# galatolofederico/clip-glass

Hardware: AMD Instinct MI355X
Metric: candidate latents scored/sec (GAN→CLIP fitness), StyleGAN2_ffhq_d pop=64 (higher is better)
Workload: dtype f16; 1 GPU; StyleGAN2_ffhq_d: StyleGAN2 config-f 1024px G+D + CLIP ViT-B/32, pop=64 per GPU, batch_size=4, n_obj=2; pop_per_gpu=64, global_pop=64, batch_size=4, parallelism=population-shard x1, device=AMD Radeon Graphics (gfx950:sramecc+:xnack-), 256 CUs, hbm_gib=288

## Files before the change

### clip_glass_amd/csrc/conv_glds.hip

```cpp
#include "common.h"
#include "kernels.h"
#include <stdlib.h>
#include <type_traits>

namespace {
constexpr int NT = 128, NTHR = 512;
template <int TW>
struct Geo {
    static constexpr int RW = TW == 32 ? 2 : 1;
    static constexpr int TH = 8 * RW * (32 / TW);
    static constexpr int PH = TH + 2, PW = TW + 2;
    static constexpr int NVA = PH * PW * 4;
    static constexpr int NA = (NVA + NTHR - 1) / NTHR;
    static constexpr int A_BYTES = NA * NTHR * 16;
    static constexpr int OFF_B = 2 * A_BYTES;
    static constexpr int OFF_C = OFF_B + 3 * (3 * NT * 64);
    static constexpr int OFF_S = OFF_C + 3 * NT * 4;
    static constexpr int OFF_T = OFF_S + 2048;
    static constexpr int OFF_N = OFF_T + 6 * NT * 2 + 512;
    static constexpr int LDS_BYTES = OFF_N + 8 * 64 * 4;
    static_assert(LDS_BYTES <= 163840, "one workgroup per CU");
};
constexpr int NB = 3 * NT * 4 / NTHR;
constexpr int B_BYTES = 3 * NT * 64;
// ... 201 lines not shown
        for (int g = 0; g < 4; ++g) {
            const int nl = j * 32 + 8 * g + 4 * kh;
            const f4 d = *(const f4*)(Cc + nl), bb = *(const f4*)(Cc + NT + nl);
#pragma unroll
            for (int i = 0; i < RW; ++i) {
                const f4 a = {acc[i][j][g * 4], acc[i][j][g * 4 + 1], acc[i][j][g * 4 + 2], acc[i][j][g * 4 + 3]};
                f4 v = act_apply(a * d + bb + nzr[i], ak);
                if (p.res) v += f4{(float)rq[g][i][0], (float)rq[g][i][1], (float)rq[g][i][2], (float)rq[g][i][3]} * p.out_scale;
                h4 out;
#pragma unroll
                for (int q = 0; q < 4; ++q) out[q] = (half_t)v[q];
                *(h4*)(Os + (i * 32 + lr) * OROW + nl * 2) = out;
                if (TRGB) va[i][g] = out;
            }
        }
        if (TRGB) {
#pragma unroll
            for (int gp = 0; gp < 2; ++gp) {
                const h8 wt = *(const h8*)(Trow + ((j * 2 + gp) * 2) * 16);
#pragma unroll
                for (int i = 0; i < RW; ++i) {
                    const h8 wi = (trow_ok && ((tn >> 2) & 1) == i) ? wt : hzero;
                    rgb = mfma32(wi, __builtin_shufflevector(va[i][2 * gp], va[i][2 * gp + 1], 0, 1, 2, 3, 4, 5, 6, 7), rgb);
                }
            }
        }
    }
    if (TRGB) {
        const long long hw = (long long)p.Ho * p.Wo;
        float* yo = p.trgb_yout + (long long)b * 3 * hw + (long long)(oyb + kh) * p.Wo + ox;
#pragma unroll
        for (int c = 0; c < 3; ++c) {
            float r = p.trgb_b[c] + (rgb[c] + rgb[4 + c] * (1.f / 2048.f));
            if (p.trgb_yprev) r += trgb_skip(ytap[c], oyb + kh, ox);
            yo[c * hw] = r;
        }
    }
    __builtin_amdgcn_wave_barrier();
#pragma unroll
    for (int i = 0; i < RW; ++i) {
#pragma unroll
        for (int k = 0; k < NT / 16; ++k) {
            const int v = lane + 64 * k;
            const int pix = v >> 4, chv = v & 15;
            const int prow = TW == 32 ? 0 : pix >> 4, pcol = TW == 32 ? pix : pix & 15;
            half_t* dst = p.y + (((long long)b * p.Ho + ty0 + (wave * RW + i) * RPL + prow) * p.Wo + tx0 + pcol) * p.Cout + n0;
            *(h8*)(dst + chv * 8) = *(const h8*)(Os + (i * 32 + pix) * OROW + chv * 16);
        }
    }
}

template <bool TRGB, bool XS = false, bool ST = true>
__global__ __launch_bounds__(512, 1) void conv_gldsp_kernel(ConvParams p, int NTn, int tiles_x, int tiles_y, int PT) {
    constexpr int TW = 32;
    using G = Geo<TW>;
    constexpr int RW = G::RW, TH = G::TH, PW = G::PW, NVA = G::NVA, NA = G::NA, A_BYTES = G::A_BYTES, OFF_B = G::OFF_B,
                  OFF_C = G::OFF_C, OFF_S = G::OFF_S;
    static_assert(RW == 2 && 8 * RW * 32 * 80 <= A_BYTES, "the sliced output image fits one patch buffer");
    static_assert(NA == 5 && NB == 3, "ring pieces per phase: one weight piece per phase of a stage, one patch piece in phases 0..4 of a chunk");
    extern __shared__ __attribute__((aligned(16))) char smem[];
    const int wave = __builtin_amdgcn_readfirstlane(threadIdx.x >> 6);
    const int grp = wave >> 2;
    const int tpi = tiles_x * tiles_y;
    const int n_work = ((PT + 7) & ~7) * NTn;
    struct Item { int b, ty0, tx0, n0, valid; };
    auto decode = [&](int id) {
        Item w;
        const int lo = id & 7, rest = id >> 3;
        const int nt = rest % NTn, pt = (rest / NTn) * 8 + lo;
        w.valid = id < n_work && pt < PT;
        const int ptc = w.valid ? pt : 0;
        w.b = ptc / tpi;
        const int trem = ptc - w.b * tpi;
        w.ty0 = (trem / tiles_x) * TH;
        w.tx0 = (trem % tiles_x) * TW;
        w.n0 = nt * NT;
        return w;
    };
    int id = blockIdx.x;
    Item cur = decode(id);
    while (id < n_work && !cur.valid) { id += gridDim.x; cur = decode(id); }
    if (id >= n_work) return;

    const half_t* xb = p.x;
    const half_t* wb = p.w;
    int a_src[NA];
    int b_src[NB];
    auto aim_a = [&](const Item& w) {
        const int t = opaque(threadIdx.x);
        xb = p.x + (long long)w.b * p.x_bstride;
#pragma unroll
        for (int k = 0; k < NA; ++k) {
            const int v = k * NTHR + t, pix = v >> 2;
            const int pr = pix / PW, pc = pix - pr * PW;
            const int iy = w.ty0 - 1 + pr, ix = w.tx0 - 1 + pc;
            const int lc = (v & 3) ^ ((pix >> 2) & 3);
            const bool ok = v < NVA && iy >= 0 && iy < p.H && ix >= 0 && ix < p.W;
            a_src[k] = ok ? (iy * p.W + ix) * p.Cin + lc * 8 : -1;
        }
    };
    auto aim_b = [&](const Item& w) {
        const int t = opaque(threadIdx.x);
        wb = p.w + (long long)w.b * p.w_bstride;
#pragma unroll
        for (int k = 0; k < NB; ++k) {
            const int v = k * NTHR + t, row = v >> 2;
            const int tx = row >> 7, n = row & 127;
            const int lc = (v & 3) ^ ((row >> 2) & 3);
            b_src[k] = (tx * p.Neff + w.n0 + n) * p.Cin + lc * 8;
        }
    };
    auto issue_a1 = [&](int k, int c, int buf) {
        char* dst = smem + buf * A_BYTES + wave * 1024 + k * (NTHR * 16);
        dma16(a_src[k] >= 0 ? xb + a_src[k] + c * 32 : g_zero_page + (threadIdx.x & 3) * 8, dst);
    };
    auto issue_b1 = [&](int k, int c, int ty, int slot) {
        char* dst = smem + OFF_B + slot * B_BYTES + wave * 1024 + k * (NTHR * 16);
        dma16(wb + (long long)ty * 3 * p.Neff * p.Cin + c * 32 + b_src[k], dst);
    };
    const int n_chunks = p.Cin >> 5;
    const half_t* Ss = (const half_t*)(smem + OFF_S);
    auto park_style = [&](int b) {
        const int t = threadIdx.x;
        if (t < (p.Cin >> 3)) *(h8*)(smem + OFF_S + t * 16) = *(const h8*)(p.sn16 + (long long)b * p.sn_stride + t * 8);
    };

    aim_a(cur);
    aim_b(cur);
    if (p.sn16) park_style(cur.b);
    {
        const int t = threadIdx.x;
        float* Cc = (float*)(smem + OFF_C);
        if (t < NT) {
            if (!p.dscale) Cc[t] = 1.f;
            if (!p.bias) Cc[NT + t] = 0.f;
            if (!p.shift) Cc[2 * NT + t] = 0.f;
        }
        if (!p.noise) *(float*)(smem + G::OFF_N + t * 4) = 0.f;
    }
    __syncthreads();
#pragma unroll
    for (int k = 0; k < NA; ++k) issue_a1(k, 0, 0);
#pragma unroll
    for (int k = 0; k < NB; ++k) issue_b1(k, 0, 0, 0);
#pragma unroll
    for (int k = 0; k < NB; ++k) issue_b1(k, 0, 1, 1);
    WAIT_VM(3);
    __builtin_amdgcn_s_barrier();
    for (;;) {
        int nid = id + gridDim.x;
        Item nxt = decode(nid);
        while (nid < n_work && !nxt.valid) { nid += gridDim.x; nxt = decode(nid); }
        const bool has_next = nid < n_work;
        if (!has_next) nxt = cur;
        const int b = cur.b, ty0 = cur.ty0, tx0 = cur.tx0, n0 = cur.n0;

        f16x acc[RW][4];
#pragma unroll
        for (int i = 0; i < RW; ++i)
#pragma unroll
            for (int j = 0; j < 4; ++j)
#pragma unroll
                for (int q = 0; q < 16; ++q) acc[i][j][q] = 0.f;

        auto prefetch_epilogue = [&]() {
            const int t = opaque(threadIdx.x), lr = t & 31, kh = (t >> 5) & 1;
            if (wave < 2) {
                char* cc = smem + OFF_C + wave * 256;
                if (p.dscale) dma4(p.dscale + (long long)b * p.ds_stride + n0 + t, cc);
                if (p.bias) dma4(p.bias + n0 + t, cc + NT * 4);
                if (p.shift) dma4(p.shift + (long long)b * p.ds_stride + n0 + t, cc + 2 * NT * 4);
            }
            if (p.noise) dma4(p.noise + ((long long)(b / p.batch_size) * p.Ho + ty0 + wave * RW + kh) * p.Wo + tx0 + lr, smem + G::OFF_N + wave * 256);
            if (TRGB && wave < 2) {
                const int row6 = min(t / (NT / 8), 5), piece = t % (NT / 8);
                const int n = row6 < 3 ? row6 : 8 + (row6 - 3);
                dma16(t < 6 * (NT / 8) ? p.trgb_tab + ((long long)b * 32 + n) * p.Neff + n0 + piece * 8 : g_zero_page, smem + G::OFF_T + wave * 1024);
            }
        };
        if (grp) __builtin_amdgcn_s_barrier();
        auto chunk_body = [&](const int c, auto lastc_tag) {
            constexpr bool lastc = decltype(lastc_tag)::value;
            const char* As = smem + (c & 1) * A_BYTES;
#pragma unroll
            for (int ty = 0; ty < 3; ++ty) {
#pragma unroll
                for (int tx = 0; tx < 3; ++tx) {
                    const int q = ty * 3 + tx;
                    auto ring_pieces = [&]() {
                        if (q == 6 && lastc) prefetch_epilogue();
                        {
                            const int t2 = (ty + 2) % 3;
                            int c2 = ty == 0 ? c : c + 1;
                            if (ty != 0 && lastc) {
                                if (q == 3) aim_b(nxt);
                                c2 = 0;
                            }
                            issue_b1(tx, c2, t2, t2);
                        }
                        if (q < 5) {
                            if (q == 0 && lastc) aim_a(nxt);
                            issue_a1(q, lastc ? 0 : c + 1, lastc ? 0 : (c + 1) & 1);
                        }
                    };
                    if (XS && q == 0 && c % NTn == (n0 >> 7)) {
                        const int tq = opaque(threadIdx.x), part = tq & 3, pix = tq >> 2, ly = pix >> 4, lx = pix & 15;
                        h8 s03, s12;
                        h8 k125, k375;
#pragma unroll
                        for (int e = 0; e < 8; ++e) { k125[e] = (half_t)0.125f; k375[e] = (half_t)0.375f; }
#pragma unroll
                        for (int jy = 0; jy < 4; ++jy) {
                            h8 a[4];
#pragma unroll
                            for (int jx = 0; jx < 4; ++jx) {
                                const int P = (2 * ly + jy) * PW + 2 * lx + jx;
                                a[jx] = *(const h8*)(As + P * 64 + ((part ^ ((P >> 2) & 3)) << 4));
                            }
                            const h8 hr = __builtin_elementwise_fma(a[0] + a[3], k125, (a[1] + a[2]) * k375);
                            if (jy == 0) s03 = hr;
                            else if (jy == 1) s12 = hr;
                            else if (jy == 2) s12 = s12 + hr;
                            else s03 = s03 + hr;
                        }
                        const h8 o = __builtin_elementwise_fma(s12, k375, s03 * k125);
                        *(h8*)(p.xs_out + (((long long)b * (p.H >> 1) + (ty0 >> 1) + ly) * (p.W >> 1) + (tx0 >> 1) + lx) * p.Cin + c * 32 + part * 8) = o;
                    }
                    h8 wf[2][4], xf[2][RW];
                    {
                        const int tm = opaque(threadIdx.x), lr = tm & 31, kh = (tm >> 5) & 1;
                        const char* Bs = smem + OFF_B + ty * B_BYTES;
#pragma unroll
                        for (int kk = 0; kk < 2; ++kk) {
                            const int lc = kk * 2 + kh;
#pragma unroll
                            for (int j = 0; j < 4; ++j) {
                                const int row = tx * NT + j * 32 + lr;
                                wf[kk][j] = *(const h8*)(Bs + row * 64 + ((lc ^ ((row >> 2) & 3)) << 4));
                            }
#pragma unroll
                            for (int i = 0; i < RW; ++i) {
                                const int pix = (wave * RW + i + ty) * PW + lr + tx;
                                xf[kk][i] = *(const h8*)(As + pix * 64 + ((lc ^ ((pix >> 2) & 3)) << 4));
                            }
                            if (ST) {
                                const h8 sv = *(const h8*)(Ss + c * 32 + lc * 8);
#pragma unroll
                                for (int j = 0; j < 4; ++j) wf[kk][j] = wf[kk][j] * sv;
                            }
                        }
                    }
                    if (tx == 2) { if (ty == 2) WAIT_VM(2); else if (ty == 1) WAIT_VM(5); else WAIT_VM(4); }
                    asm volatile("s_waitcnt lgkmcnt(0)" ::: "memory");
                    __builtin_amdgcn_sched_barrier(0);
                    __builtin_amdgcn_s_barrier();
                    __builtin_amdgcn_s_setprio(1);
#pragma unroll
                    for (int kk = 0; kk < 2; ++kk)
#pragma unroll
                        for (int j = 0; j < 4; ++j) {
#pragma unroll
                            for (int i = 0; i < RW; ++i) acc[i][j] = mfma32(wf[kk][j], xf[kk][i], acc[i][j]);
                            if (kk == 0 && j == 1) { __builtin_amdgcn_sched_barrier(0); ring_pieces(); __builtin_amdgcn_sched_barrier(0); }
                        }
                    __builtin_amdgcn_s_setprio(0);
                    __builtin_amdgcn_sched_barrier(0);
                    __builtin_amdgcn_s_barrier();
                }
            }
        };
        for (int c = 0; c + 1 < n_chunks; ++c) chunk_body(c, std::false_type{});
        chunk_body(n_chunks - 1, std::true_type{});

        if (!grp) __builtin_amdgcn_s_barrier();
        const int t = opaque(threadIdx.x), lane = t & 63, lr = lane & 31, kh = lane >> 5;
        const float* Cc = (const float*)(smem + OFF_C);
        constexpr int OP = 80;
        char* Os = smem + A_BYTES + wave * (RW * 32 * OP);
        const int oyb = ty0 + wave * RW, ox = tx0 + lr;
        const int rcs = p.res_cs ? p.res_cs : p.Cout;
        const ActK ak = act_consts(p.act, p.out_scale);
        float ytap[3][4];
        h8 nsty;
        if (TRGB && p.trgb_yprev) {
            const int my = (oyb + kh) >> 1, mx = ox >> 1, h2 = p.Ho >> 1, w2 = p.Wo >> 1;
            const float* yp = p.trgb_yprev + (long long)b * 3 * h2 * w2;
#pragma unroll
            for (int cc = 0; cc < 3; ++cc)
#pragma unroll
                for (int q = 0; q < 4; ++q)
                    ytap[cc][q] = yp[(cc * h2 + max(my - 1 + (q >> 1), 0)) * w2 + max(mx - 1 + (q & 1), 0)];
        }
        if (ST && t < (p.Cin >> 3)) nsty = *(const h8*)(p.sn16 + (long long)nxt.b * p.sn_stride + t * 8);
        float nzr[RW];
#pragma unroll
        for (int i = 0; i < RW; ++i) nzr[i] = p.noise_strength * *(const float*)(smem + G::OFF_N + (wave * 64 + i * 32 + lr) * 4);
        f16x rgb;
#pragma unroll
        for (int q = 0; q < 16; ++q) rgb[q] = 0.f;
        const int tn = lr & 15;
        const char* Trow = smem + G::OFF_T + (((tn >> 3) & 1) * 3 + min(tn & 3, 2)) * (NT * 2) + kh * 16;
        const bool trow_ok = (tn & 3) < 3;
        const h8 hzero = {0, 0, 0, 0, 0, 0, 0, 0};
#pragma unroll
        for (int j = 0; j < 4; ++j) {
            h4 va[RW][4];
            h4 rq[4][RW];
            if (p.res) {
#pragma unroll
                for (int i = 0; i < RW; ++i) {
                    const int oy = oyb + i;
                    const half_t* rp = p.res + (p.res_up ? (((long long)b * (p.Ho >> 1) + (oy >> 1)) * (p.Wo >> 1) + (ox >> 1)) * rcs
                                                         : (((long long)b * p.Ho + oy) * p.Wo + ox) * rcs) + n0 + j * 32 + 4 * kh;
#pragma unroll
                    for (int g = 0; g < 4; ++g) rq[g][i] = *(const h4*)(rp + 8 * g);
                }
            }
            constexpr int GB = TRGB ? 2 : 4;
#pragma unroll
            for (int g0 = 0; g0 < 4; g0 += GB) {
            f4 dq[GB], bq[GB];
#pragma unroll
            for (int g = 0; g < GB; ++g) {
                const int nl = j * 32 + 8 * (g0 + g) + 4 * kh;
                dq[g] = *(const f4*)(Cc + nl);
                bq[g] = *(const f4*)(Cc + NT + nl) + *(const f4*)(Cc + 2 * NT + nl);
            }
            __builtin_amdgcn_sched_barrier(0);
#pragma unroll
            for (int g = g0; g < g0 + GB; ++g) {
                const f4 d = dq[g - g0], bb = bq[g - g0];
#pragma unroll
                for (int i = 0; i < RW; ++i) {
                    const f4 a = {acc[i][j][g * 4], acc[i][j][g * 4 + 1], acc[i][j][g * 4 + 2], acc[i][j][g * 4 + 3]};
                    f4 v = act_apply(a * d + bb + nzr[i], ak);
                    if (p.res) v += f4{(float)rq[g][i][0], (float)rq[g][i][1], (float)rq[g][i][2], (float)rq[g][i][3]} * p.out_scale;
                    h4 out;
#pragma unroll
                    for (int q = 0; q < 4; ++q) out[q] = (half_t)v[q];
                    *(h4*)(Os + (i * 32 + lr) * OP + (8 * g + 4 * kh) * 2) = out;
                    if (TRGB) va[i][g] = out;
                }
            }
            }
            if (TRGB) {
#pragma unroll
                for (int gp = 0; gp < 2; ++gp) {
                    const h8 wt = *(const h8*)(Trow + ((j * 2 + gp) * 2) * 16);
#pragma unroll
                    for (int i = 0; i < RW; ++i) {
                        const h8 wi = (trow_ok && ((tn >> 2) & 1) == i) ? wt : hzero;
                        rgb = mfma32(wi, __builtin_shufflevector(va[i][2 * gp], va[i][2 * gp + 1], 0, 1, 2, 3, 4, 5, 6, 7), rgb);
                    }
                }
            }
            __builtin_amdgcn_wave_barrier();
#pragma unroll
            for (int k = 0; k < 4; ++k) {
                const int v = lane + 64 * k, i = v >> 7, pix = (v >> 2) & 31, piece = v & 3;
                half_t* dst = p.y + (((long long)b * p.Ho + oyb + i) * p.Wo + tx0 + pix) * p.Cout + n0 + j * 32 + piece * 8;
                *(h8*)dst = *(const h8*)(Os + (i * 32 + pix) * OP + piece * 16);
            }
            __builtin_amdgcn_wave_barrier();
        }
        if (TRGB) {
            const long long hw = (long long)p.Ho * p.Wo;
            if (p.trgb_part) {
                float* yo = p.trgb_part + ((long long)(n0 >> 7) * p.B + b) * 3 * hw + (long long)(oyb + kh) * p.Wo + ox;
#pragma unroll
                for (int cc = 0; cc < 3; ++cc) yo[cc * hw] = rgb[cc] + rgb[4 + cc] * (1.f / 2048.f);
            } else {
                float* yo = p.trgb_yout + (long long)b * 3 * hw + (long long)(oyb + kh) * p.Wo + ox;
#pragma unroll
                for (int cc = 0; cc < 3; ++cc) {
                    float r = p.trgb_b[cc] + (rgb[cc] + rgb[4 + cc] * (1.f / 2048.f));
                    if (p.trgb_yprev) r += trgb_skip(ytap[cc], oyb + kh, ox);
                    yo[cc * hw] = r;
                }
            }
        }
        if (ST && t < (p.Cin >> 3)) *(h8*)(smem + OFF_S + t * 16) = nsty;
        asm volatile("s_waitcnt lgkmcnt(0)" ::: "memory");
        __builtin_amdgcn_s_barrier();
        if (!has_next) break;
        id = nid;
        cur = nxt;
    }
    WAIT_VM(0);
}


static constexpr uint32_t GLDS_FEATURES = CF_STYLE | CF_DEMOD | CF_SHIFT | CF_NOISE | CF_RES | CF_RES_CS | CF_RES_UP | CF_SAMPLE_W | CF_TORGB |
                                          CF_TORGB_PART | CF_XS_OUT;

static int glds_cus() { return glass_cu_count() - glass_cu_count() % 8; }
template <int TW, bool TRGB>
static void launch_glds(const ConvParams& p, hipStream_t st) {
    using G = Geo<TW>;
    static DevOnce once;
    once.run([&] { (void)hipFuncSetAttribute((const void*)conv_glds_kernel<TW, TRGB>, hipFuncAttributeMaxDynamicSharedMemorySize, G::LDS_BYTES); });
    const int tiles_x = p.Wc / TW, tiles_y = p.Hc / G::TH, PT = p.B * tiles_x * tiles_y, NTn = p.Neff / NT;
    hipLaunchKernelGGL((conv_glds_kernel<TW, TRGB>), dim3((PT + 7) / 8 * 8 * NTn), dim3(NTHR), G::LDS_BYTES, st, p, NTn, tiles_x, tiles_y, PT);
}
template <bool TRGB, bool XS, bool ST>
static void launch_gldsp(const ConvParams& p, hipStream_t st) {
    using G = Geo<32>;
    static DevOnce once;
    once.run([&] { (void)hipFuncSetAttribute((const void*)conv_gldsp_kernel<TRGB, XS, ST>, hipFuncAttributeMaxDynamicSharedMemorySize, G::LDS_BYTES); });
    const int tiles_x = p.Wc / 32, tiles_y = p.Hc / G::TH, PT = p.B * tiles_x * tiles_y, NTn = p.Neff / NT;
    hipLaunchKernelGGL((conv_gldsp_kernel<TRGB, XS, ST>), dim3(glds_cus()), dim3(NTHR), G::LDS_BYTES, st, p, NTn, tiles_x, tiles_y, PT);
}

template <int TW, bool TRGB = false>
static ConvKernel glds_inst(const ConvParams& p, const char* name) {
    const long long work_nominal = (long long)GLASS_NOMINAL_POP * (p.Wc / TW) * (p.Hc / Geo<TW>::TH) * (p.Neff / NT);
    if (TW == 32 && (p.Cin & 63) == 0 && work_nominal >= 2 * glds_cus()) {
        const bool sty = p.sn16 != nullptr;
        if (p.xs_out && !TRGB) return sty ? ConvKernel{"conv_gldsp_kernel<false,true,true>", launch_gldsp<false, true, true>}
                                          : ConvKernel{"conv_gldsp_kernel<false,true,false>", launch_gldsp<false, true, false>};
        if (TRGB) return sty ? ConvKernel{"conv_gldsp_kernel<true,false,true>", launch_gldsp<true, false, true>}
                             : ConvKernel{"conv_gldsp_kernel<true,false,false>", launch_gldsp<true, false, false>};
        return sty ? ConvKernel{"conv_gldsp_kernel<false,false,true>", launch_gldsp<false, false, true>}
                   : ConvKernel{"conv_gldsp_kernel<false,false,false>", launch_gldsp<false, false, false>};
    }
    if (p.xs_out || p.trgb_part) return conv_refused();
    return {name, launch_glds<TW, TRGB>};
}

ConvKernel choose_conv_glds(const ConvParams& p) {
    const uint32_t f = conv_features(p);
    if (f & ~GLDS_FEATURES) return conv_refused(f & ~GLDS_FEATURES);
    if (!glass_lds_fits(Geo<32>::LDS_BYTES) || !glass_lds_fits(Geo<16>::LDS_BYTES)) return conv_refused();
    if (((f & CF_XS_OUT) && ((f & (CF_STYLE | CF_TORGB | CF_TORGB_PART)) || p.Wc % 32 != 0)) || !p.y || p.KS != 3 || p.stride != 1 || p.pad != 1)
        return conv_refused();
    if (((f & CF_STYLE) && !p.sn16) || p.Cin > 1024) return conv_refused();
    if (p.Cin % 32 != 0 || p.Cin < 128 || p.Neff % NT != 0 || (p.Cout & 7) || p.Hc % 16 != 0) return conv_refused();
    if ((long long)p.H * p.W * p.Cin >= (1LL << 31)) return conv_refused();
    if (f & CF_TORGB_PART) {
        if (!p.trgb_tab || (f & CF_TORGB) || p.trgb_yprev || p.Neff != p.Cout || p.Wc % 32 != 0) return conv_refused();
        return glds_inst<32, true>(p, nullptr);
    }
    if (f & CF_TORGB) {
        if (!p.trgb_tab || !p.trgb_b || p.Neff != NT || p.Cout != NT || p.Wc % 32 != 0) return conv_refused();
        return glds_inst<32, true>(p, "conv_glds_kernel<32,true>");
    }
    if (p.Wc % 32 == 0) return glds_inst<32>(p, "conv_glds_kernel<32>");
    if (p.Wc % 16 == 0) return glds_inst<16>(p, "conv_glds_kernel<16>");
    return conv_refused();
}
```

### clip_glass_amd/csrc/conv_stream.hip

```cpp
#include "common.h"
#include "kernels.h"
#include <stdio.h>
#include <stdlib.h>

namespace {
constexpr int TH = 8, PH = TH + 2;
constexpr int W_BYTES = 9 * 32 * 64;
constexpr int PP = 36;
constexpr int A_BYTES = PH * PP * 64;
constexpr int O_BYTES = 4 * 32 * 64;
constexpr int C_BYTES = 32 * 4 + 32 * 4 + 32 * 2 + 4 * 32 * 2;
constexpr int LDS_BYTES = W_BYTES + A_BYTES + O_BYTES + C_BYTES;
__device__ __forceinline__ int swz(int row, int chunk) { return (row << 6) + ((chunk ^ ((row >> 2) & 3)) << 4); }
__device__ __forceinline__ int opaque(int v) { asm volatile("" : "+v"(v)); return v; }
__device__ __forceinline__ int swa(int pr, int pc, int chunk) { return ((pr * PP + pc) << 6) + ((chunk ^ ((pc >> 2) & 3)) << 4); }
}

template <bool FRGB, bool TRGB, bool TR = false>
__global__ __launch_bounds__(256, 3) void conv_stream_kernel(ConvParams p, int tiles_x, int tiles_y, int PT, int per_block) {
    static_assert(!TR, "placeholder of a removed experiment");
    extern __shared__ __attribute__((aligned(16))) char smem[];
    char* Ws = smem;
    char* As = smem + W_BYTES;
    const int t = threadIdx.x;
    float* Cd = (float*)(smem + W_BYTES + A_BYTES + O_BYTES);
    float* Cb = Cd + 32;
    half_t* Cs = (half_t*)(Cb + 32);
    half_t* Cf = Cs + 32;
    char* Tw = smem + W_BYTES + A_BYTES;
    float* Ys = (float*)(Tw + 2048);
    float* Tb = Ys + 256;
    if (FRGB) {
        if (t < 32) {
            Cf[t] = (half_t)(p.rgb_w[t * 3] * GLASS_SQRT2);
            Cf[32 + t] = (half_t)(p.rgb_w[t * 3 + 1] * GLASS_SQRT2);
            Cf[64 + t] = (half_t)(p.rgb_w[t * 3 + 2] * GLASS_SQRT2);
            Cf[96 + t] = (half_t)(p.rgb_b[t] * GLASS_SQRT2);
        }
        __syncthreads();
    }

    const int first = blockIdx.x * per_block;
    const int last = min(first + per_block, PT);
    if (first >= last) return;

    struct Cur { int b, ty, tx; };
    auto cur_at = [&](int id) {
        Cur c;
        const int tpi = tiles_x * tiles_y;
        c.b = id / tpi;
        const int trem = id - c.b * tpi;
        if (p.row_walk) { c.ty = trem / tiles_x; c.tx = trem - c.ty * tiles_x; }
        else { c.tx = trem / tiles_y; c.ty = trem - c.tx * tiles_y; }
        return c;
    };
    auto advance = [&](Cur& c) {
        if (p.row_walk) {
            if (++c.tx == tiles_x) { c.tx = 0; if (++c.ty == tiles_y) { c.ty = 0; ++c.b; } }
        } else if (++c.ty == tiles_y) {
            c.ty = 0;
            if (++c.tx == tiles_x) { c.tx = 0; ++c.b; }
        }
    };
    const Cur c_first = cur_at(first);
    auto pick = [&](const Cur& c, bool live) {
        Cur r;
        r.b = live ? c.b : c_first.b; r.ty = live ? c.ty : c_first.ty; r.tx = live ? c.tx : c_first.tx;
        return r;
    };
#define GEO(tt)                                                                                                       \
    const int hi = __builtin_amdgcn_readfirstlane((tt) >> 7);                                                          \
    const unsigned tbyte = (unsigned)((tt) & 127) * 16u;                                                                \
    const int bpc = (((tt) >> 2) & 31) + 1;                                                                             \
    const int lbody = swa(hi, bpc, (tt) & 3);                                                                           \
    const int hpr = (tt) >> 3, hpc = (((tt) >> 2) & 1) * 33;                                                            \
    const int lhalo = swa(hpr, hpc, (tt) & 3);                                                                          \
    const int f1r = (tt) < 64 ? 8 + ((tt) >> 5) : ((tt) - 64) >> 1, f1c = (tt) < 64 ? ((tt) & 31) + 1 : (((tt) - 64) & 1) * 33; \
    (void)hi; (void)tbyte; (void)bpc; (void)lbody; (void)hpr; (void)hpc; (void)lhalo; (void)f1r; (void)f1c

    struct RSet { h8 a[FRGB ? 1 : 6]; float y3[FRGB ? 2 : 1][3]; float nz[2]; float ys[TRGB ? 3 : 1]; };
    auto load_part = [&](const Cur& c, RSet& R, int k) {
        const int ty0 = c.ty * TH, tx0 = c.tx * 32;
        const int t = opaque(threadIdx.x);
        GEO(t);
        if (FRGB) {
            const int hw = p.H * p.W;
            const float* yb = p.rgb_y + (long long)c.b * 3 * hw;
            if (k == 0 || (k == 1 && t < 84)) {
                const int pr = k ? f1r : (t >> 5), pc = k ? f1c : (t & 31) + 1;
                const int iy = min(max(ty0 - 1 + pr, 0), p.H - 1), ix = min(max(tx0 - 1 + pc, 0), p.W - 1);
                const int off = iy * p.W + ix;
#pragma unroll
                for (int ch = 0; ch < 3; ++ch) R.y3[k][ch] = yb[ch * hw + off];
            }
        } else {
            const half_t* img = p.x + (long long)c.b * p.x_bstride;
            if (k < 5) {
                const int row = min(max(ty0 - 1 + 2 * k + hi, 0), p.H - 1);
                const char* rowp = (const char*)(img + ((long long)row * p.W + tx0) * 32);
                R.a[k] = *(const h8*)(rowp + tbyte);
            } else if (k == 5) {
                if (t < 80) {
                    const int iy = min(max(ty0 - 1 + hpr, 0), p.H - 1), ix = min(max(tx0 - 1 + hpc, 0), p.W - 1);
                    R.a[5] = *(const h8*)(img + ((long long)iy * p.W + ix) * 32 + (t & 3) * 8);
                }
            }
        }
        if (k == 6) {
            if (p.noise) {
                const float* nzp = p.noise + ((long long)(c.b / p.batch_size) * p.Ho + ty0) * p.Wo + tx0;
                const int noff = ((t >> 6) & 3) * 2 * p.Wo + (t & 31);
                R.nz[0] = nzp[noff];
                R.nz[1] = nzp[noff + p.Wo];
            }
            if (TRGB && p.trgb_yprev) {
                const int r = t >> 5, col = t & 31;
                if (r < 5 && col < 17) {
                    const int h2 = p.Ho >> 1, w2 = p.Wo >> 1;
                    const int sy = max((ty0 >> 1) - 1 + r, 0), sx = max((tx0 >> 1) - 1 + col, 0);
                    const float* yp = p.trgb_yprev + (long long)c.b * 3 * h2 * w2 + sy * w2 + sx;
#pragma unroll
                    for (int ch = 0; ch < 3; ++ch) R.ys[ch] = yp[ch * h2 * w2];
                }
            }
        }
    };
    auto load = [&](const Cur& c, RSet& R) {
#pragma unroll
        for (int k = 0; k <= 6; ++k) load_part(c, R, k);
    };

    int wb = -1;
    auto step = [&](int id, const Cur& cc, const Cur& lc, RSet& R) {
        const bool valid = id < last;
        const int b = cc.b, ty0 = cc.ty * TH, tx0 = cc.tx * 32;
        __syncthreads();
        if (wb != b && (TRGB || wb < 0 || p.w_bstride != 0 || p.dscale || p.shift || p.sn16)) {
            const half_t* wsrc = p.w + (long long)b * p.w_bstride;
            for (int u = t; u < 9 * 32 * 4; u += 256)
                *(h8*)(Ws + swz(u >> 2, u & 3)) = *(const h8*)(wsrc + (long long)(u >> 2) * 32 + (u & 3) * 8);
            if (t < 32) {
                Cd[t] = p.dscale ? p.dscale[(long long)b * p.ds_stride + t] : 1.f;
                Cb[t] = (p.bias ? p.bias[t] : 0.f) + (p.shift ? p.shift[(long long)b * p.ds_stride + t] : 0.f);
                Cs[t] = p.sn16 ? p.sn16[(long long)b * p.sn_stride + t] : (half_t)1.f;
            }
            if (TRGB) {
                const float sm = p.trgb_smax[(long long)b * p.trgb_smax_stride];
#pragma unroll
                for (int u = 0; u < 4; ++u) {
                    const int e = t + 256 * u, tab = e >> 9, n = (e >> 5) & 15, hidx = e & 31;
                    const int col = n & 3, j = hidx & 7;
                    const int ch = 8 * (2 * (hidx >> 4) + (j >> 2)) + 4 * ((hidx >> 3) & 1) + (j & 3);
                    half_t val = (half_t)0.f;
                    if (col < 3 && ((n >> 2) & 1) == tab) {
                        const float w = p.trgb_w[col * 32 + ch] * p.trgb_sn[(long long)b * p.trgb_sn_stride + ch] * sm;
                        const half_t hv = (half_t)w;
                        val = (n & 8) ? (half_t)((w - (float)hv) * 2048.f) : hv;
                    }
                    ((half_t*)Tw)[e] = val;
                }
                if (t < 3) Tb[t] = p.trgb_b[t];
            }
            wb = b;
            __syncthreads();
        }
        const int t = opaque(threadIdx.x);
        GEO(t);
        const bool border = ty0 == 0 || tx0 == 0 || ty0 + TH >= p.H || tx0 + 32 >= p.W;
        const h8 zero = {0, 0, 0, 0, 0, 0, 0, 0};
        if (FRGB) {
            h8 fw[4][4];
#pragma unroll
            for (int part = 0; part < 4; ++part)
#pragma unroll
                for (int r = 0; r < 4; ++r) fw[part][r] = *(const h8*)(Cf + r * 32 + part * 8);
            auto pixel = [&](int k, bool masked) {
                const int pr = k ? f1r : (t >> 5), pc = k ? f1c : (t & 31) + 1;
                const int iy = ty0 - 1 + pr, ix = tx0 - 1 + pc;
                float c3[3];
#pragma unroll
                for (int ch = 0; ch < 3; ++ch) c3[ch] = fminf(fmaxf((R.y3[k][ch] + 1.f) * 0.5f, 0.f), 1.f) * 2.f - 1.f;
                const half_t h0 = (half_t)c3[0], h1 = (half_t)c3[1], h2 = (half_t)c3[2];
                const int lrow = (pr * PP + pc) << 6, key = (pc >> 2) & 3;
                h8 a[4];
#pragma unroll
                for (int part = 0; part < 4; ++part) {
                    const h8 z = fw[part][0] * h0 + fw[part][1] * h1 + fw[part][2] * h2 + fw[part][3];
                    a[part] = __builtin_elementwise_max(z, z * (half_t)0.2f);
                }
                if (p.rgb_x_out && valid && pr >= 1 && pr <= TH && pc >= 1 && pc <= 32) {
                    half_t* xo = p.rgb_x_out + (((long long)b * p.H + iy) * p.W + ix) * 32;
#pragma unroll
                    for (int part = 0; part < 4; ++part) *(h8*)(xo + part * 8) = a[part];
                }
                const bool ok = !masked || (iy >= 0 && iy < p.H && ix >= 0 && ix < p.W);
#pragma unroll
                for (int part = 0; part < 4; ++part) *(h8*)(As + lrow + ((part ^ key) << 4)) = ok ? a[part] : zero;
            };
            if (border) {
                pixel(0, true);
                if (t < 84) pixel(1, true);
            } else {
                pixel(0, false);
                if (t < 84) pixel(1, false);
            }
        } else {
            if (!border && !p.sn16) {
#pragma unroll
                for (int k = 0; k < 5; ++k) *(h8*)(As + lbody + k * (2 * PP * 64)) = R.a[k];
                if (t < 80) *(h8*)(As + lhalo) = R.a[5];
            } else {
                const h8 sh = *(const h8*)(Cs + (t & 3) * 8);
#pragma unroll
                for (int k = 0; k < 5; ++k) {
                    h8 a = R.a[k];
                    if (border && (unsigned)(ty0 - 1 + 2 * k + hi) >= (unsigned)p.H) a = zero;
                    *(h8*)(As + lbody + k * (2 * PP * 64)) = a * sh;
                }
                if (t < 80) {
                    h8 a = R.a[5];
                    if (border && ((unsigned)(ty0 - 1 + hpr) >= (unsigned)p.H || (unsigned)(tx0 - 1 + hpc) >= (unsigned)p.W)) a = zero;
                    *(h8*)(As + lhalo) = a * sh;
                }
            }
        }
        if (TRGB && p.trgb_yprev) {
            const int r = t >> 5, col = t & 31;
            if (r < 5 && col < 17) {
                const bool ok = (ty0 >> 1) - 1 + r >= 0 && (tx0 >> 1) - 1 + col >= 0;
#pragma unroll
                for (int ch = 0; ch < 3; ++ch) Ys[ch * 85 + r * 17 + col] = ok ? R.ys[ch] : 0.f;
            }
        }
        __syncthreads();
        const float nz0 = p.noise ? p.noise_strength * R.nz[0] : 0.f, nz1 = p.noise ? p.noise_strength * R.nz[1] : 0.f;

        f16x acc[2];
#pragma unroll
        for (int i = 0; i < 2; ++i)
#pragma unroll
            for (int q = 0; q < 16; ++q) acc[i][q] = 0.f;
        const int tm = opaque(threadIdx.x), lr = tm & 31, kh = (tm >> 5) & 1, wave = tm >> 6, lane = tm & 63;
        char* Os = smem + W_BYTES + A_BYTES + wave * (32 * 64);
        __builtin_amdgcn_s_setprio(1);
#pragma unroll
        for (int ty = 0; ty < 3; ++ty)
#pragma unroll
            for (int tx = 0; tx < 3; ++tx) {
                const int tap = ty * 3 + tx;
                if (tap <= 6) load_part(lc, R, tap);
#pragma unroll
                for (int kk = 0; kk < 2; ++kk) {
                    const h8 wf = *(const h8*)(Ws + swz(tap * 32 + lr, kk * 2 + kh));
#pragma unroll
                    for (int i = 0; i < 2; ++i) {
                        const h8 xf = *(const h8*)(As + swa(wave * 2 + i + ty, lr + tx, kk * 2 + kh));
                        acc[i] = mfma32(wf, xf, acc[i]);
                    }
                }
            }
        __builtin_amdgcn_s_setprio(0);
        if (FRGB && p.rgb_xs_out && valid) {
            const int tx_ = opaque(threadIdx.x), part = tx_ & 3;
            const int pix = tx_ >> 2, ly = pix >> 4, lx = pix & 15;
            h8 hr[4];
#pragma unroll
            for (int jy = 0; jy < 4; ++jy) {
                const int pr = 2 * ly + jy, pc = 2 * lx;
                const h8 a0 = *(const h8*)(As + swa(pr, pc, part)), a1 = *(const h8*)(As + swa(pr, pc + 1, part)),
                         a2 = *(const h8*)(As + swa(pr, pc + 2, part)), a3 = *(const h8*)(As + swa(pr, pc + 3, part));
                hr[jy] = (a0 + a3) * (half_t)0.125f + (a1 + a2) * (half_t)0.375f;
            }
            const h8 o = (hr[0] + hr[3]) * (half_t)0.125f + (hr[1] + hr[2]) * (half_t)0.375f;
            *(h8*)(p.rgb_xs_out + (((long long)b * (p.H >> 1) + (ty0 >> 1) + ly) * (p.W >> 1) + (tx0 >> 1) + lx) * 32 + part * 8) = o;
        }
        const half_t k1 = (half_t)((p.act == 1 ? GLASS_SQRT2 : 1.f) * p.out_scale);
        const half_t k2 = (half_t)((p.act == 1 ? 0.2f * GLASS_SQRT2 : p.act == 2 ? 0.f : 1.f) * p.out_scale);
        if (TRGB) {
            f16x rgb;
#pragma unroll
            for (int q = 0; q < 16; ++q) rgb[q] = 0.f;
#pragma unroll
            for (int i = 0; i < 2; ++i) {
                const float nz = i ? nz1 : nz0;
                h4 va[4];
#pragma unroll
                for (int g = 0; g < 4; ++g) {
                    const int o = 8 * g + 4 * kh;
                    const f4 d = *(const f4*)(Cd + o), bb = *(const f4*)(Cb + o);
                    h4 v;
#pragma unroll
                    for (int q = 0; q < 4; ++q) v[q] = (half_t)(acc[i][g * 4 + q] * d[q] + (nz + bb[q]));
                    va[g] = __builtin_elementwise_max(v * k1, v * k2);
                }
                const char* Tt = Tw + i * 1024 + (lr & 15) * 64 + kh * 16;
                rgb = mfma32(*(const h8*)Tt, __builtin_shufflevector(va[0], va[1], 0, 1, 2, 3, 4, 5, 6, 7), rgb);
                rgb = mfma32(*(const h8*)(Tt + 32), __builtin_shufflevector(va[2], va[3], 0, 1, 2, 3, 4, 5, 6, 7), rgb);
            }
            float r3[3];
#pragma unroll
            for (int ch = 0; ch < 3; ++ch) r3[ch] = Tb[ch] + (rgb[ch] + rgb[4 + ch] * (1.f / 2048.f));
            if (p.trgb_yprev) {
                const float wy0 = kh ? 0.25f : 0.75f, wx0 = (lr & 1) ? 0.25f : 0.75f;
                const float* yw = Ys + wave * 17 + (lr >> 1);
#pragma unroll
                for (int ch = 0; ch < 3; ++ch) {
                    float sacc = 0.f;
                    sacc += wy0 * wx0 * yw[ch * 85];
                    sacc += wy0 * (1.f - wx0) * yw[ch * 85 + 1];
                    sacc += (1.f - wy0) * wx0 * yw[ch * 85 + 17];
                    sacc += (1.f - wy0) * (1.f - wx0) * yw[ch * 85 + 18];
                    r3[ch] += sacc;
                }
            }
            if (valid) {
                const long long hw = (long long)p.Ho * p.Wo;
                float* yo = p.trgb_yout + (long long)b * 3 * hw + (long long)(ty0 + wave * 2 + kh) * p.Wo + tx0 + lr;
#pragma unroll
                for (int ch = 0; ch < 3; ++ch) yo[ch * hw] = r3[ch];
            }
        } else {
#pragma unroll
            for (int i = 0; i < 2; ++i) {
                const int oy = ty0 + wave * 2 + i;
                const float nz = i ? nz1 : nz0;
#pragma unroll
                for (int g = 0; g < 4; ++g) {
                    const int o = 8 * g + 4 * kh;
                    const f4 d = *(const f4*)(Cd + o), bb = *(const f4*)(Cb + o);
                    h4 v;
#pragma unroll
                    for (int q = 0; q < 4; ++q) v[q] = (half_t)(acc[i][g * 4 + q] * d[q] + (nz + bb[q]));
                    *(h4*)(Os + swz(lr, o >> 3) + (o & 4) * 2) = __builtin_elementwise_max(v * k1, v * k2);
                }
                __builtin_amdgcn_wave_barrier();
                if (valid) {
                    half_t* yrow = p.y + (((long long)b * p.Ho + oy) * p.Wo + tx0) * 32;
#pragma unroll
                    for (int k = 0; k < 2; ++k) {
                        const int v = lane + 64 * k;
                        *(h8*)(yrow + (long long)(v >> 2) * 32 + (v & 3) * 8) = *(const h8*)(Os + swz(v >> 2, v & 3));
                    }
                }
                __builtin_amdgcn_wave_barrier();
            }
        }
    };

    RSet r0, r1;
    Cur cc = c_first, lc = c_first;
    load(pick(lc, true), r0);
    advance(lc);
    load(pick(lc, first + 1 < last), r1);
    advance(lc);
    for (int id = first; id < last; id += 2) {
        step(id, pick(cc, true), pick(lc, id + 2 < last), r0);
        advance(cc); advance(lc);
        step(id + 1, pick(cc, id + 1 < last), pick(lc, id + 3 < last), r1);
        advance(cc); advance(lc);
    }
}

static int stream_slots() {
    static DevOnce once;
    once.run([&] {
        (void)hipFuncSetAttribute((const void*)conv_stream_kernel<false, false, false>, hipFuncAttributeMaxDynamicSharedMemorySize, LDS_BYTES);
        (void)hipFuncSetAttribute((const void*)conv_stream_kernel<true, false, false>, hipFuncAttributeMaxDynamicSharedMemorySize, LDS_BYTES);
        (void)hipFuncSetAttribute((const void*)conv_stream_kernel<false, true, false>, hipFuncAttributeMaxDynamicSharedMemorySize, LDS_BYTES);
    });
    return glass_cu_count() * 3;
}

static constexpr uint32_t STREAM_FEATURES = CF_STYLE | CF_DEMOD | CF_SHIFT | CF_NOISE | CF_SAMPLE_W | CF_BCAST_X | CF_FROMRGB | CF_TORGB | CF_NO_MAP;

template <bool FRGB, bool TRGB>
static void launch_stream(const ConvParams& p0, hipStream_t st) {
    ConvParams p = p0;
    p.row_walk = FRGB ? 1 : 0;
    const int tiles_x = p.Wc / 32, tiles_y = p.Hc / TH;
    const int PT = p.B * tiles_x * tiles_y;
    const int slots = stream_slots();
    const int per_block = (PT + slots - 1) / slots;
    const int grid = (PT + per_block - 1) / per_block;
    hipLaunchKernelGGL((conv_stream_kernel<FRGB, TRGB, false>), dim3(grid), dim3(256), LDS_BYTES, st, p, tiles_x, tiles_y, PT, per_block);
}

ConvKernel choose_conv_stream(const ConvParams& p) {
    const uint32_t f = conv_features(p);
    if (f & ~STREAM_FEATURES) return conv_refused(f & ~STREAM_FEATURES);
    const bool trgb = f & CF_TORGB, frgb = f & CF_FROMRGB;
    if (trgb != !p.y) return conv_refused();
    if (!glass_lds_fits(LDS_BYTES)) return conv_refused();
    if (p.KS != 3 || p.stride != 1 || p.pad != 1 || ((f & CF_STYLE) && !p.sn16)) return conv_refused();
    if (frgb && (!p.rgb_w || !p.rgb_b || (!p.rgb_x_out && !p.rgb_xs_out) || (f & (CF_STYLE | CF_TORGB | CF_SHIFT)))) return conv_refused();
    if (trgb && (!p.trgb_w || !p.trgb_b || !p.trgb_sn || !p.trgb_smax || p.Ho != p.Hc || p.Wo != p.Wc)) return conv_refused();
    if (p.Cin != 32 || p.Neff != 32 || p.Cout != 32) return conv_refused();
    if (p.Wc % 32 != 0 || p.Hc % TH != 0 || p.W >= 256 * 32 || (!frgb && (f & CF_BCAST_X))) return conv_refused();
    if ((long long)p.H * p.W * p.Cin >= (1LL << 31)) return conv_refused();
    const long long PT_nominal = (long long)GLASS_NOMINAL_POP * (p.Wc / 32) * (p.Hc / TH);
    if (PT_nominal < (long long)stream_slots() * 6) return conv_refused();
    if (frgb) return {"conv_stream_kernel<fromrgb>", launch_stream<true, false>};
    if (trgb) return {"conv_stream_kernel<torgb>", launch_stream<false, true>};
    return {"conv_stream_kernel", launch_stream<false, false>};
}
```

Measured before the change: 2289 candidates/s.

## Software-pipeline conv epilogue slices and specialize lean path without residual/demod

Restructures the per-slice epilogue so the next slice's activation math overlaps with the LDS transpose and global stores of the current one, using sched barriers to order them. It also dispatches to a lean specialization that skips the demod scale, the second bias load and the residual loads when the layer has no residual, dscale or shift, and drops the noise add when none is used. The cost is higher register pressure from the packed outputs and read buffers, plus extra template instantiations.

```diff
diff --git a/clip_glass_amd/csrc/conv_glds.hip b/clip_glass_amd/csrc/conv_glds.hip
--- a/clip_glass_amd/csrc/conv_glds.hip
+++ b/clip_glass_amd/csrc/conv_glds.hip
@@ -527,11 +527,15 @@
         const char* Trow = smem + G::OFF_T + (((tn >> 3) & 1) * 3 + min(tn & 3, 2)) * (NT * 2) + kh * 16;
         const bool trow_ok = (tn & 3) < 3;
         const h8 hzero = {0, 0, 0, 0, 0, 0, 0, 0};
-#pragma unroll
-        for (int j = 0; j < 4; ++j) {
-            h4 va[RW][4];
+        char* const ybase = (char*)(p.y + (((long long)b * p.Ho + oyb) * p.Wo + tx0) * p.Cout + n0);
+        const unsigned yoff = ((lane >> 2) * p.Cout + (lane & 3) * 8) * 2;
+        auto run_slices = [&](auto lean_tag, auto nz_tag) {
+        constexpr bool LEAN = decltype(lean_tag)::value, NZ = decltype(nz_tag)::value;
+        h4 pk[RW][4];
+        h8 rd[4];
+        auto slice_valu = [&](const int j) {
             h4 rq[4][RW];
-            if (p.res) {
+            if (!LEAN && p.res) {
 #pragma unroll
                 for (int i = 0; i < RW; ++i) {
                     const int oy = oyb + i;
@@ -540,6 +544,11 @@
 #pragma unroll
                     for (int g = 0; g < 4; ++g) rq[g][i] = *(const h4*)(rp + 8 * g);
                 }
+            } else if (!LEAN) {
+#pragma unroll
+                for (int i = 0; i < RW; ++i)
+#pragma unroll
+                    for (int g = 0; g < 4; ++g) rq[g][i] = h4{0, 0, 0, 0};
             }
             constexpr int GB = TRGB ? 2 : 4;
 #pragma unroll
@@ -548,6 +557,7 @@
 #pragma unroll
             for (int g = 0; g < GB; ++g) {
                 const int nl = j * 32 + 8 * (g0 + g) + 4 * kh;
+                if (LEAN) { bq[g] = *(const f4*)(Cc + NT + nl); continue; }
                 dq[g] = *(const f4*)(Cc + nl);
                 bq[g] = *(const f4*)(Cc + NT + nl) + *(const f4*)(Cc + 2 * NT + nl);
             }
@@ -558,13 +568,15 @@
 #pragma unroll
                 for (int i = 0; i < RW; ++i) {
                     const f4 a = {acc[i][j][g * 4], acc[i][j][g * 4 + 1], acc[i][j][g * 4 + 2], acc[i][j][g * 4 + 3]};
-                    f4 v = act_apply(a * d + bb + nzr[i], ak);
-                    if (p.res) v += f4{(float)rq[g][i][0], (float)rq[g][i][1], (float)rq[g][i][2], (float)rq[g][i][3]} * p.out_scale;
+                    f4 v = act_apply(LEAN ? (NZ ? a + bb + nzr[i] : a + bb) : a * d + bb + nzr[i], ak);
+                    if (!LEAN) {
+                        const f4 vr = v + f4{(float)rq[g][i][0], (float)rq[g][i][1], (float)rq[g][i][2], (float)rq[g][i][3]} * p.out_scale;
+                        v = p.res ? vr : v;
+                    }
                     h4 out;
 #pragma unroll
                     for (int q = 0; q < 4; ++q) out[q] = (half_t)v[q];
-                    *(h4*)(Os + (i * 32 + lr) * OP + (8 * g + 4 * kh) * 2) = out;
-                    if (TRGB) va[i][g] = out;
+                    pk[i][g] = out;
                 }
             }
             }
@@ -575,19 +587,36 @@
 #pragma unroll
                     for (int i = 0; i < RW; ++i) {
                         const h8 wi = (trow_ok && ((tn >> 2) & 1) == i) ? wt : hzero;
-                        rgb = mfma32(wi, __builtin_shufflevector(va[i][2 * gp], va[i][2 * gp + 1], 0, 1, 2, 3, 4, 5, 6, 7), rgb);
+                        rgb = mfma32(wi, __builtin_shufflevector(pk[i][2 * gp], pk[i][2 * gp + 1], 0, 1, 2, 3, 4, 5, 6, 7), rgb);
                     }
                 }
             }
+        };
+        slice_valu(0);
+#pragma unroll
+        for (int j = 0; j < 4; ++j) {
+            __builtin_amdgcn_sched_barrier(0);
+#pragma unroll
+            for (int g = 0; g < 4; ++g)
+#pragma unroll
+                for (int i = 0; i < RW; ++i) *(h4*)(Os + (i * 32 + lr) * OP + (8 * g + 4 * kh) * 2) = pk[i][g];
             __builtin_amdgcn_wave_barrier();
 #pragma unroll
             for (int k = 0; k < 4; ++k) {
                 const int v = lane + 64 * k, i = v >> 7, pix = (v >> 2) & 31, piece = v & 3;
-                half_t* dst = p.y + (((long long)b * p.Ho + oyb + i) * p.Wo + tx0 + pix) * p.Cout + n0 + j * 32 + piece * 8;
-                *(h8*)dst = *(const h8*)(Os + (i * 32 + pix) * OP + piece * 16);
-            }
-            __builtin_amdgcn_wave_barrier();
-        }
+                rd[k] = *(const h8*)(Os + (i * 32 + pix) * OP + piece * 16);
+            }
+            __builtin_amdgcn_sched_barrier(0);
+            if (j < 3) slice_valu(j + 1);
+            __builtin_amdgcn_sched_barrier(0);
+#pragma unroll
+            for (int k = 0; k < 4; ++k)
+                *(h8*)(ybase + ((long long)(k >> 1) * p.Wo + 16 * (k & 1)) * p.Cout * 2 + j * 64 + yoff) = rd[k];
+        }
+        };
+        if (p.res || p.dscale || p.shift) run_slices(std::false_type{}, std::true_type{});
+        else if (TRGB || p.noise) run_slices(std::true_type{}, std::true_type{});
+        else run_slices(std::true_type{}, std::false_type{});
         if (TRGB) {
             const long long hw = (long long)p.Ho * p.Wo;
             if (p.trgb_part) {
```

Result: no change. 2302 candidates/s, median of 6 (+0.6%).

## Hoist LDS/global address bases and add resident-weight fast path in conv stream

Applied to the files above, without the earlier changes.

Precomputes per-thread LDS fragment bases and global row offsets once per kernel and per tile, using scalar base plus unsigned 32-bit offsets for global loads. It replaces row clamping with edge adjustments. It also reuses the loaded activation rows across the three vertical taps, so the inner MFMA loop needs fewer LDS reads. A compile-time RESTAGE flag adds an inner loop that skips the weight-restage check when the weights for consecutive tiles are already resident. This cuts VALU address math, LDS traffic and branching, at the cost of more live registers (18 h8 fragments) that could reduce occupancy.

```diff
diff --git a/clip_glass_amd/csrc/conv_stream.hip b/clip_glass_amd/csrc/conv_stream.hip
--- a/clip_glass_amd/csrc/conv_stream.hip
+++ b/clip_glass_amd/csrc/conv_stream.hip
@@ -2,6 +2,7 @@
 #include "kernels.h"
 #include <stdio.h>
 #include <stdlib.h>
+#include <type_traits>
 
 namespace {
 constexpr int TH = 8, PH = TH + 2;
@@ -70,20 +71,38 @@
     };
 #define GEO(tt)                                                                                                       \
     const int hi = __builtin_amdgcn_readfirstlane((tt) >> 7);                                                          \
-    const unsigned tbyte = (unsigned)((tt) & 127) * 16u;                                                                \
     const int bpc = (((tt) >> 2) & 31) + 1;                                                                             \
     const int lbody = swa(hi, bpc, (tt) & 3);                                                                           \
     const int hpr = (tt) >> 3, hpc = (((tt) >> 2) & 1) * 33;                                                            \
     const int lhalo = swa(hpr, hpc, (tt) & 3);                                                                          \
     const int f1r = (tt) < 64 ? 8 + ((tt) >> 5) : ((tt) - 64) >> 1, f1c = (tt) < 64 ? ((tt) & 31) + 1 : (((tt) - 64) & 1) * 33; \
-    (void)hi; (void)tbyte; (void)bpc; (void)lbody; (void)hpr; (void)hpc; (void)lhalo; (void)f1r; (void)f1c
+    (void)hi; (void)bpc; (void)lbody; (void)hpr; (void)hpc; (void)lhalo; (void)f1r; (void)f1c
+
+    const int tg = opaque(threadIdx.x);
+    int wbase[2], pbase[3][2];
+#pragma unroll
+    for (int kk = 0; kk < 2; ++kk) {
+        wbase[kk] = opaque(swz(tg & 31, kk * 2 + ((tg >> 5) & 1)));
+#pragma unroll
+        for (int tx = 0; tx < 3; ++tx) pbase[tx][kk] = opaque(swa((tg >> 6) * 2, (tg & 31) + tx, kk * 2 + ((tg >> 5) & 1)));
+    }
+    const unsigned lbyte = (unsigned)opaque((tg & 127) * 16);
 
     struct RSet { h8 a[FRGB ? 1 : 6]; float y3[FRGB ? 2 : 1][3]; float nz[2]; float ys[TRGB ? 3 : 1]; };
-    auto load_part = [&](const Cur& c, RSet& R, int k) {
+    struct LBase { const char* img; unsigned off; int r0; };
+    auto load_base = [&](const Cur& c) {
+        LBase L;
+        const int hi = __builtin_amdgcn_readfirstlane(opaque(threadIdx.x) >> 7);
+        L.img = FRGB ? nullptr : (const char*)(p.x + (long long)c.b * p.x_bstride);
+        L.r0 = c.ty * TH - 1 + hi;
+        L.off = (unsigned)(L.r0 * p.W + c.tx * 32) * 64u;
+        return L;
+    };
+    auto load_part = [&](const Cur& c, const LBase& L, unsigned tbyte, RSet& R, int k) {
         const int ty0 = c.ty * TH, tx0 = c.tx * 32;
-        const int t = opaque(threadIdx.x);
-        GEO(t);
         if (FRGB) {
+            const int t = opaque(threadIdx.x);
+            GEO(t);
             const int hw = p.H * p.W;
             const float* yb = p.rgb_y + (long long)c.b * 3 * hw;
             if (k == 0 || (k == 1 && t < 84)) {
@@ -94,48 +113,60 @@
                 for (int ch = 0; ch < 3; ++ch) R.y3[k][ch] = yb[ch * hw + off];
             }
         } else {
-            const half_t* img = p.x + (long long)c.b * p.x_bstride;
             if (k < 5) {
-                const int row = min(max(ty0 - 1 + 2 * k + hi, 0), p.H - 1);
-                const char* rowp = (const char*)(img + ((long long)row * p.W + tx0) * 32);
-                R.a[k] = *(const h8*)(rowp + tbyte);
+                const unsigned pitch = (unsigned)p.W * 64u;
+                unsigned o = L.off + (unsigned)(2 * k) * pitch;
+                if (k == 0) o += L.r0 < 0 ? pitch : 0u;
+                if (k == 4) o -= L.r0 + 8 >= p.H ? pitch : 0u;
+                unsigned long long rowp = (unsigned long long)(L.img + o);
+                asm volatile("" : "+s"(rowp));
+                R.a[k] = *(const __attribute__((address_space(1))) h8*)(rowp + tbyte);
             } else if (k == 5) {
+                const int t = opaque(threadIdx.x);
                 if (t < 80) {
+                    const int hpr = t >> 3, hpc = ((t >> 2) & 1) * 33;
                     const int iy = min(max(ty0 - 1 + hpr, 0), p.H - 1), ix = min(max(tx0 - 1 + hpc, 0), p.W - 1);
-                    R.a[5] = *(const h8*)(img + ((long long)iy * p.W + ix) * 32 + (t & 3) * 8);
+                    R.a[5] = *(const h8*)(L.img + ((unsigned)(iy * p.W + ix) * 64u + (unsigned)(t & 3) * 16u));
                 }
             }
         }
         if (k == 6) {
+            const int t = opaque(threadIdx.x);
             if (p.noise) {
                 const float* nzp = p.noise + ((long long)(c.b / p.batch_size) * p.Ho + ty0) * p.Wo + tx0;
-                const int noff = ((t >> 6) & 3) * 2 * p.Wo + (t & 31);
-                R.nz[0] = nzp[noff];
-                R.nz[1] = nzp[noff + p.Wo];
+                const unsigned noff = (unsigned)(((t >> 6) & 3) * 2 * p.Wo + (t & 31)) * 4u;
+                R.nz[0] = *(const float*)((const char*)nzp + noff);
+                R.nz[1] = *(const float*)((const char*)(nzp + p.Wo) + noff);
             }
             if (TRGB && p.trgb_yprev) {
                 const int r = t >> 5, col = t & 31;
                 if (r < 5 && col < 17) {
                     const int h2 = p.Ho >> 1, w2 = p.Wo >> 1;
                     const int sy = max((ty0 >> 1) - 1 + r, 0), sx = max((tx0 >> 1) - 1 + col, 0);
-                    const float* yp = p.trgb_yprev + (long long)c.b * 3 * h2 * w2 + sy * w2 + sx;
-#pragma unroll
-                    for (int ch = 0; ch < 3; ++ch) R.ys[ch] = yp[ch * h2 * w2];
+                    const float* yp = p.trgb_yprev + (long long)c.b * 3 * h2 * w2;
+                    const unsigned yoff = (unsigned)(sy * w2 + sx) * 4u;
+#pragma unroll
+                    for (int ch = 0; ch < 3; ++ch) R.ys[ch] = *(const float*)((const char*)(yp + (long long)ch * h2 * w2) + yoff);
                 }
             }
         }
     };
     auto load = [&](const Cur& c, RSet& R) {
-#pragma unroll
-        for (int k = 0; k <= 6; ++k) load_part(c, R, k);
+        const LBase L = load_base(c);
+#pragma unroll
+        for (int k = 0; k <= 6; ++k) load_part(c, L, lbyte, R, k);
     };
 
     int wb = -1;
-    auto step = [&](int id, const Cur& cc, const Cur& lc, RSet& R) {
+    const bool per_sample = TRGB || p.w_bstride != 0 || p.dscale || p.shift || p.sn16;
+    auto stale = [&](int b) { return wb < 0 || (per_sample && wb != b); };
+    auto step = [&](auto may_restage, int id, const Cur& cc, const Cur& lc, RSet& R) {
+        constexpr bool RESTAGE = decltype(may_restage)::value;
         const bool valid = id < last;
         const int b = cc.b, ty0 = cc.ty * TH, tx0 = cc.tx * 32;
         __syncthreads();
-        if (wb != b && (TRGB || wb < 0 || p.w_bstride != 0 || p.dscale || p.shift || p.sn16)) {
+        if (RESTAGE && stale(b)) {
+            const int t = opaque(threadIdx.x);
             const half_t* wsrc = p.w + (long long)b * p.w_bstride;
             for (int u = t; u < 9 * 32 * 4; u += 256)
                 *(h8*)(Ws + swz(u >> 2, u & 3)) = *(const h8*)(wsrc + (long long)(u >> 2) * 32 + (u & 3) * 8);
@@ -233,32 +264,35 @@
             }
         }
         __syncthreads();
-        const float nz0 = p.noise ? p.noise_strength * R.nz[0] : 0.f, nz1 = p.noise ? p.noise_strength * R.nz[1] : 0.f;
-
-        f16x acc[2];
-#pragma unroll
-        for (int i = 0; i < 2; ++i)
-#pragma unroll
-            for (int q = 0; q < 16; ++q) acc[i][q] = 0.f;
+        typedef float f2 __attribute__((ext_vector_type(2)));
+        const float nzs0 = p.noise ? p.noise_strength * R.nz[0] : 0.f, nzs1 = p.noise ? p.noise_strength * R.nz[1] : 0.f;
+        f2 nzp0 = {nzs0, nzs0}, nzp1 = {nzs1, nzs1};
+        asm volatile("" : "+v"(nzp0), "+v"(nzp1));
+        const float nz0 = nzp0[0], nz1 = nzp1[0];
+
         const int tm = opaque(threadIdx.x), lr = tm & 31, kh = (tm >> 5) & 1, wave = tm >> 6, lane = tm & 63;
         char* Os = smem + W_BYTES + A_BYTES + wave * (32 * 64);
+        const LBase L = load_base(lc);
+        const unsigned lb = (unsigned)opaque((int)lbyte);
+        f16x acc[2];
+        h8 x1[18];
         __builtin_amdgcn_s_setprio(1);
 #pragma unroll
-        for (int ty = 0; ty < 3; ++ty)
-#pragma unroll
-            for (int tx = 0; tx < 3; ++tx) {
-                const int tap = ty * 3 + tx;
-                if (tap <= 6) load_part(lc, R, tap);
-#pragma unroll
-                for (int kk = 0; kk < 2; ++kk) {
-                    const h8 wf = *(const h8*)(Ws + swz(tap * 32 + lr, kk * 2 + kh));
-#pragma unroll
-                    for (int i = 0; i < 2; ++i) {
-                        const h8 xf = *(const h8*)(As + swa(wave * 2 + i + ty, lr + tx, kk * 2 + kh));
-                        acc[i] = mfma32(wf, xf, acc[i]);
-                    }
-                }
-            }
+        for (int g = 0; g < 18; ++g) {
+            const int ty = g / 6, tx = (g >> 1) % 3, kk = g & 1, tap = g >> 1;
+            if (!kk && tap <= 6) load_part(lc, L, lb, R, tap);
+            const h8 wf = *(const h8*)(Ws + wbase[kk] + tap * 2048);
+            x1[g] = *(const h8*)(As + pbase[tx][kk] + (1 + ty) * (PP * 64));
+            const h8 x0 = ty == 0 ? *(const h8*)(As + pbase[tx][kk]) : x1[g < 6 ? 0 : g - 6];
+            if (g == 0) {
+                const f16x z = {0.f, 0.f, 0.f, 0.f, 0.f, 0.f, 0.f, 0.f, 0.f, 0.f, 0.f, 0.f, 0.f, 0.f, 0.f, 0.f};
+                acc[0] = mfma32(wf, x0, z);
+                acc[1] = mfma32(wf, x1[g], z);
+            } else {
+                acc[0] = mfma32(wf, x0, acc[0]);
+                acc[1] = mfma32(wf, x1[g], acc[1]);
+            }
+        }
         __builtin_amdgcn_s_setprio(0);
         if (FRGB && p.rgb_xs_out && valid) {
             const int tx_ = opaque(threadIdx.x), part = tx_ & 3;
@@ -315,9 +349,10 @@
             }
             if (valid) {
                 const long long hw = (long long)p.Ho * p.Wo;
-                float* yo = p.trgb_yout + (long long)b * 3 * hw + (long long)(ty0 + wave * 2 + kh) * p.Wo + tx0 + lr;
-#pragma unroll
-                for (int ch = 0; ch < 3; ++ch) yo[ch * hw] = r3[ch];
+                float* yo = p.trgb_yout + (long long)b * 3 * hw + (long long)ty0 * p.Wo + tx0;
+                const unsigned ooff = (unsigned)((wave * 2 + kh) * p.Wo + lr) * 4u;
+#pragma unroll
+                for (int ch = 0; ch < 3; ++ch) *(float*)((char*)(yo + ch * hw) + ooff) = r3[ch];
             }
         } else {
 #pragma unroll
@@ -353,11 +388,24 @@
     advance(lc);
     load(pick(lc, first + 1 < last), r1);
     advance(lc);
-    for (int id = first; id < last; id += 2) {
-        step(id, pick(cc, true), pick(lc, id + 2 < last), r0);
+    const std::true_type general;
+    const std::false_type resident;
+    for (int id = first; id < last;) {
+        step(general, id, pick(cc, true), pick(lc, id + 2 < last), r0);
         advance(cc); advance(lc);
-        step(id + 1, pick(cc, id + 1 < last), pick(lc, id + 3 < last), r1);
+        step(general, id + 1, pick(cc, id + 1 < last), pick(lc, id + 3 < last), r1);
         advance(cc); advance(lc);
+        id += 2;
+        for (;;) {
+            Cur c1 = cc;
+            advance(c1);
+            if (id + 1 >= last || stale(cc.b) || stale(c1.b)) break;
+            step(resident, id, cc, pick(lc, id + 2 < last), r0);
+            advance(cc); advance(lc);
+            step(resident, id + 1, cc, pick(lc, id + 3 < last), r1);
+            advance(cc); advance(lc);
+            id += 2;
+        }
     }
 }
 
```

Result: no change. 2295 candidates/s before, 2304 candidates/s after, median of 6 (+0.4%).
